# skeskinen/bert.cpp

Hardware: AMD Instinct MI355X
Metric: sentences/sec (seq_len=128) (higher is better)
Workload: dtype f16; 1 GPU; all-MiniLM-L6-v2 f16, batch=256 seq_len=128; per_gpu_batch=256, global_batch=256, seq_len=128, weights=f16, parallelism=dp1 (replicated weights, sharded sentences)

## Files before the change

bert.cpp_amd/csrc/engine.hip:

```cpp
#include "engine.h"

#include <algorithm>
#include <cstdio>
#include <cstdlib>
#include <chrono>
#include <cstring>
#include <system_error>
#include <thread>

namespace bert_hip {

Engine *Engine::create(const ModelFile &mf, int device, std::string &err) {
    int ndev = 0;
    if (hipGetDeviceCount(&ndev) != hipSuccess || ndev <= 0) {
        err = "no HIP device available (this library needs an AMD GPU; there is no CPU fallback)";
        return nullptr;
    }
    if (device < 0 || device >= ndev) { err = "HIP device ordinal " + std::to_string(device) + " out of range"; return nullptr; }
    std::unique_ptr<Engine> e(new Engine);
    e->hp_ = mf.hp;
    e->device_ = device;
    if (hipSetDevice(e->device_) != hipSuccess) { err = "hipSetDevice failed"; return nullptr; }
    hipDeviceProp_t prop;
    if (hipGetDeviceProperties(&prop, e->device_) != hipSuccess) { err = "hipGetDeviceProperties failed"; return nullptr; }
// ... 11 lines not shown
    return e.release();
}

Engine::~Engine() {
    (void)hipSetDevice(device_);
    (void)hipDeviceSynchronize();
    for (auto &sl : slot_) {
        if (sl.h_in) (void)hipHostFree(sl.h_in);
        if (sl.h_out) (void)hipHostFree(sl.h_out);
        if (sl.done) (void)hipEventDestroy(sl.done);
    }
    if (busy_) (void)hipEventDestroy(busy_);
    if (stream_) (void)hipStreamDestroy(stream_);
}

bool Engine::reserve(int n_tokens, int n_sentences, std::string &err) {
    HIP_OK(hipSetDevice(device_), err, false);
    if (n_tokens <= 0 || n_sentences <= 0) return true;
    return ensure_workspace((n_tokens + 255) / 256 * 256, n_sentences, err);
}

int Engine::check(std::string &err) {
    HIP_OK(hipSetDevice(device_), err, -1);
    HIP_OK(hipDeviceSynchronize(), err, -1);
    int st = 0;
    HIP_OK(hipMemcpy(&st, status_.p, sizeof(int), hipMemcpyDeviceToHost), err, -1);
    if (st) HIP_OK(hipMemset(status_.p, 0, sizeof(int)), err, -1);
    return st;
}

void Engine::set_option(const std::string &key, const std::string &value) {
    if (key == "profile_replay") { prof_.set_replay(value); return; }
    (void)hipSetDevice(device_);
    if (!test_poison_option(key, ctx_)) opt_.set(key, value, w_->naive_images(), w_->fold_images);
}

bool Engine::ensure_workspace(int t_pad, int n_sentences, std::string &err) {
    const size_t H = hp_.n_embd, I = hp_.n_intermediate, tp = (size_t)t_pad;
    const size_t es = w_->f32_file ? 4 : 2;
    return x_.ensure(tp * H * es, err) && qkv_.ensure(tp * 3 * H * es, err) && ctx_.ensure(tp * H * es, err) &&
           y_.ensure(tp * H * es, err) && ff_.ensure(tp * I * es, err) && v32_.ensure((size_t)std::max(128, std::min(t_pad, (opt_.latency_tokens + 255) / 256 * 256)) * H * 4, err) &&
           d_out_.ensure((size_t)n_sentences * H * 4, err) &&
           windows_.ensure((size_t)n_sentences * sizeof(int2), err) &&
           (!(H > 384 && H % 256 == 0) || (ln_stats1_.ensure(tp * (2 * H / 256) * 8, err) && ln_stats2_.ensure(tp * (2 * H / 256) * 8, err) &&
                                           ln_rows1_.ensure(tp * 16, err) && ln_rows2_.ensure(tp * 16, err)));
}

void Engine::timed_launch(const char *name, double flops, hipStream_t s, const std::function<void()> &f) { timed(name, flops, s, f); }

std::string Engine::profile_report() {
    (void)hipSetDevice(device_);
    (void)hipDeviceSynchronize();
    return prof_.report();
}

void Engine::build_windows(const int32_t *cu, int B, std::vector<int2> &windows, int slot) {
    windows.clear();
    int first = 0, fill = 0;
    for (int b = 0; b < B; ++b) {
        const int n = cu[b + 1] - cu[b];
        if (b > first && fill + n > 128) {
            windows.push_back(make_int2(first, b - first));
            first = b; fill = 0;
        }
        fill = (fill + n + slot - 1) & ~(slot - 1);
    }
    if (B > first) windows.push_back(make_int2(first, B - first));
// ... 117 lines not shown
    float *v32 = v32_.as<float>();
    for (int il = 0; il < Lz; ++il) {
        const LayerWeights &L = w_->layers[il];
        const LayerWeights *P = il ? &w_->layers[il - 1] : nullptr;
        timed("skinny_qkv", 2.0 * p.T * 3 * H * H, p.s, [&] {
            launch_skinny_gemm(0, L.qkv.w, x, P ? v32 : nullptr, P ? P->ln_out_w.as<float>() : nullptr, P ? P->ln_out_b.as<float>() : nullptr,
                               x, L.qkv_b.as<float>(), nullptr, qkv, nullptr, tb, p.s);
        });
        attention(p);
        timed("skinny_proj", 2.0 * p.T * H * H, p.s, [&] {
            launch_skinny_gemm(1, L.o.w, ctx, nullptr, nullptr, nullptr, nullptr, L.o_b.as<float>(), x, nullptr, v32, tb, p.s);
        });
        timed("skinny_ffn_up", 2.0 * p.T * H * I, p.s, [&] {
            launch_skinny_gemm(2, L.ffi.w, nullptr, v32, L.ln_att_w.as<float>(), L.ln_att_b.as<float>(), y, L.ffi_b.as<float>(), nullptr, ff, nullptr, tb, p.s);
        });
        timed("skinny_ffn_down", 2.0 * p.T * H * I, p.s, [&] {
            launch_skinny_gemm(3, L.ffo.w, ff, nullptr, nullptr, nullptr, nullptr, L.ffo_b.as<float>(), y, nullptr, v32, tb, p.s);
        });
        if (il + 1 == Lz || p.hidden)
            timed("skinny_layernorm", 0.0, p.s, [&] { launch_skinny_layernorm(v32, L.ln_out_w.as<float>(), L.ln_out_b.as<float>(), x, tb, H, p.s); });
        tap(p, il + 1);
    }
}

void Engine::forward_one_launch(const Plan &p) {
    const int H = hp_.n_embd, I = hp_.n_intermediate;
    ModelLayerWeights mw[MODEL_MAX_LAYERS];
    for (int il = 0; il < hp_.n_layer; ++il) {
        const LayerWeights &L = w_->layers[il];
        mw[il] = {&L.qkv.w, &L.o.w, &L.ffi.w, &L.ffo.w, L.qkv_b.as<float>(), L.o_b.as<float>(), L.ln_att_w.as<float>(), L.ln_att_b.as<float>(),
                  L.ffi_b.as<float>(), L.ffo_b.as<float>(), L.ln_out_w.as<float>(), L.ln_out_b.as<float>()};
    }
    timed("model_kernel", hp_.n_layer * (2.0 * p.T * 3 * H * H + 4.0 * p.T * p.max_len * H + 2.0 * p.T * H * H + 4.0 * p.T * H * I), p.s, [&] {
        launch_model_kernel(mw, hp_.n_layer, x_.as<half_t>(), ctx_.as<half_t>(), p.cu, p.B, p.T, p.windows, p.n_windows, p.n_windows_dev, hp_.n_head,
                            p.out, p.max_len, status_.as<int>(), p.pool_mode, p.slots, p.s);
    });
}

bool Engine::forward_folded(const Plan &p, std::string &err) {
    const int H = hp_.n_embd, P = 2 * H / 256;
    const Family G = Family::GEMM256;
    half_t *x = x_.as<half_t>(), *qkv = qkv_.as<half_t>(), *ctx = ctx_.as<half_t>(), *y = y_.as<half_t>(), *ff = ff_.as<half_t>();
    float2 *st1 = ln_stats1_.as<float2>(), *st2 = ln_stats2_.as<float2>();
    float4 *rows1 = ln_rows1_.as<float4>(), *rows2 = ln_rows2_.as<float4>();
    for (int il = 0; il < hp_.n_layer; ++il) {
        const LayerWeights &L = w_->layers[il];
        GemmLnFold ln;
        if (il == 0) {
            if (!gemm(p, "gemm_qkv", G, p.layers[0].planes ? L.qkv_q4 : L.qkv, x, L.qkv_b.as<float>(), nullptr, qkv, EPI_BIAS, err)) return false;
        } else {
            ln.flags = GemmLnFold::IN; ln.rows_in = rows2; ln.waug = L.qkv_waug.as<half_t>();
            if (!gemm(p, "gemm_qkv", G, L.qkv_fold, x, nullptr, nullptr, qkv, EPI_BIAS, err, &ln)) return false;
        }
        attention(p);
        ln = GemmLnFold(); ln.flags = GemmLnFold::STATS | (il ? GemmLnFold::RES : 0); ln.stats = st1; ln.rows_res = rows2; ln.gb = L.o_gb.as<unsigned>();
        if (!gemm(p, "gemm_attn_out", G, L.o, ctx, L.o_b.as<float>(), x, y, EPI_BIAS_RESID, err, &ln)) return false;
        timed("ln_rows_finalize", 0.0, p.s, [&] { launch_ln_rows_finalize(st1, P, p.t_pad, H, rows1, p.s); });
        ln = GemmLnFold(); ln.flags = GemmLnFold::IN; ln.rows_in = rows1; ln.waug = L.ffi_waug.as<half_t>();
        if (!gemm(p, "gemm_ffn_up", G, L.ffi_fold, y, nullptr, nullptr, ff, EPI_BIAS_GELU, err, &ln)) return false;
        ln = GemmLnFold(); ln.flags = GemmLnFold::STATS | GemmLnFold::RES; ln.stats = st2; ln.rows_res = rows1; ln.gb = L.ffo_gb.as<unsigned>();
        if (!gemm(p, "gemm_ffn_down", G, L.ffo, ff, L.ffo_b.as<float>(), y, x, EPI_BIAS_RESID, err, &ln)) return false;
        timed("ln_rows_finalize", 0.0, p.s, [&] { launch_ln_rows_finalize(st2, P, p.t_pad, H, rows2, p.s); });
        if (il + 1 == hp_.n_layer)
            timed("layernorm", 0.0, p.s, [&] { launch_layernorm(x, L.ln_out_w.as<float>(), L.ln_out_b.as<float>(), p.T, H, p.s); });
    }
    return true;
}
// ... 209 lines not shown
```

bert.cpp_amd/csrc/kernels.h:

```cpp
#pragma once
#include <hip/hip_runtime.h>
#include <hip/hip_ext.h>

#include <atomic>
#include <cstdint>
#include <thread>

namespace bert_hip {

typedef _Float16 half_t;

constexpr int GEMM_BM = 128;
constexpr int GEMM_BN = 128;
constexpr int GEMM_BK = 64;

enum Epilogue : int { EPI_BIAS = 0, EPI_BIAS_GELU = 1, EPI_BIAS_RESID = 2 };
enum GemmWType : int { GW_F16 = 0, GW_Q4_0 = 1, GW_Q4_1 = 2 };

struct GemmWeight {
    int N = 0, K = 0, N_pad = 0;
    int type = GW_F16;
    const half_t *w16 = nullptr;
    const uint4 *qs = nullptr;
    const void *sc = nullptr;
    const half_t *naive16 = nullptr;
    const half_t *w16p = nullptr;
    const float *w32 = nullptr;
};

void launch_gemm_mfma(const GemmWeight &W, const half_t *A, const float *bias, const half_t *resid, half_t *C,
                      int M_pad, int epilogue, hipStream_t stream);
bool gemm256_supported(const GemmWeight &W, int M_pad);
struct GemmLnFold {
    enum : int { IN = 1, RES = 2, STATS = 4 };
    int flags = 0;
    const float4 *rows_in = nullptr;
    const half_t *waug = nullptr;
    const float4 *rows_res = nullptr;
    const unsigned *gb = nullptr;
    float2 *stats = nullptr;
};
bool launch_gemm256(const GemmWeight &W, const half_t *A, const float *bias, const half_t *resid, half_t *C, int M_pad,
                    int epilogue, hipStream_t stream, const GemmLnFold *ln = nullptr);
void launch_ln_rows_finalize(const float2 *stats, int P, int T, int H, float4 *rows, hipStream_t stream);
bool layer_tail_supported(const GemmWeight &Wo, const GemmWeight &W1, const GemmWeight &W2);
void launch_layer_tail(const GemmWeight &Wo, const GemmWeight &W1, const GemmWeight &W2, const half_t *ctx, const half_t *x,
                       const float *bo, const float *g1, const float *be1, const float *b1, const float *b2,
                       const float *g2, const float *be2, half_t *out, int M_pad, hipStream_t stream);
constexpr int MODEL_MAX_LAYERS = 12;
struct ModelLayerWeights {
    const GemmWeight *Wqkv, *Wo, *W1, *W2;
    const float *bqkv, *bo, *g1, *be1, *b1, *b2, *g2, *be2;
};
bool model_kernel_supported(const GemmWeight &Wqkv, const GemmWeight &Wo, const GemmWeight &W1, const GemmWeight &W2, int n_layer,
                            int n_head, int d_head, int max_len);
void launch_model_kernel(const ModelLayerWeights *layers, int n_layer, half_t *x, half_t *ctx, const int32_t *cu_seqlens, int n_sentences,
                         int n_tokens, const int2 *groups, int n_groups, const int *n_groups_dev, int n_head, float *pooled, int max_len,
                         int *status, int pool_mode, int slots, hipStream_t stream);
bool skinny_layer_supported(const GemmWeight &Wqkv, const GemmWeight &Wo, const GemmWeight &W1, const GemmWeight &W2);
void launch_skinny_gemm(int mode, const GemmWeight &W, const half_t *A, const float *V, const float *gamma, const float *beta,
                        half_t *ln_out, const float *bias, const half_t *resid, half_t *out16, float *out32, int n_token_blocks,
                        hipStream_t stream);
void launch_skinny_layernorm(const float *v, const float *gamma, const float *beta, half_t *out, int n_token_blocks, int H,
                             hipStream_t stream);
void launch_gemm_naive(const GemmWeight &W, const half_t *A, const float *bias, const half_t *resid, half_t *C,
                       int M, int epilogue, hipStream_t stream);

void launch_embed_ln(const void *word, const void *type, const void *pos, int table_type, const float *gamma,
                     const float *beta, const int32_t *tokens, const int32_t *cu_seqlens, int n_sentences, int T,
                     int H, int n_vocab, int max_len, half_t *out, hipStream_t stream);

void launch_layernorm(half_t *x, const float *gamma, const float *beta, int T, int H, hipStream_t stream);

bool launch_attention_mfma(const half_t *qkv, const int32_t *cu_seqlens, int n_sentences, int n_head, int d_head,
                           int max_len, half_t *out, hipStream_t stream);
void launch_attention_naive(const half_t *qkv, const int32_t *cu_seqlens, int n_sentences, int n_head, int d_head,
                            int max_len, half_t *out, hipStream_t stream);

bool qkv_attention2_supported(const GemmWeight &Wqkv, int n_head, int d_head, int max_len);
int qkv_attention2_sentences_per_window(int max_len, int slots);
void launch_qkv_attention2(const GemmWeight &Wqkv, const half_t *x, const float *bias, const int32_t *cu_seqlens,
                           int n_sentences, const int2 *groups, int n_groups, const int *n_groups_dev, int max_len, int n_head,
                           int slots, half_t *out, hipStream_t stream);
void launch_build_windows(const int32_t *cu_seqlens, int n_sentences, int2 *windows, int *n_windows, int slots, hipStream_t stream);
int qkv_attention2_max_windows(int n_sentences, int n_tokens, int slots);
int window_slots();
void set_window_slots(int slots);

constexpr int POOL_CLS = 1, POOL_RAW = 2;
// ... 51 lines not shown
```

bert.cpp_amd/csrc/layer_tail.hip:

```cpp
#include "device.h"

namespace bert_hip {

namespace {

constexpr int LT_TILE = 16384;
#ifndef LT_ABLATE
#define LT_ABLATE 0
#endif
#ifndef LT_UPRIO
#define LT_UPRIO 1
#endif
#ifndef LT_GELU_BATCH
#define LT_GELU_BATCH 0
#endif
#ifndef LT_DMA_SPLIT
#define LT_DMA_SPLIT 1
#endif
#ifndef LT_DPRIO
#define LT_DPRIO 0
#endif

#ifdef BERT_HIP_TIMELINE
static __device__ unsigned long long g_tl_tail[256 * 512];
// ... 25 lines not shown
    asm volatile("s_waitcnt lgkmcnt(%4)" : "+v"(f[0]), "+v"(f[1]), "+v"(f[2]), "+v"(f[3]) : "n"(N) : "memory");
}
template <int N>
__device__ __forceinline__ void wait_lgkm() {
    asm volatile("s_waitcnt lgkmcnt(%0)" : : "n"(N) : "memory");
}
template <int VM>
__device__ __forceinline__ void close_interval(f16x8 (&f)[4]) {
    asm volatile("s_waitcnt vmcnt(%4) lgkmcnt(0)\n\ts_barrier" : "+v"(f[0]), "+v"(f[1]), "+v"(f[2]), "+v"(f[3]) : "n"(VM) : "memory");
}
template <int OFF>
__device__ __forceinline__ f16x8 frag_read(unsigned addr) {
    if (LT_ABLATE & 4) { f16x8 z = (f16x8)(_Float16)0.f; asm volatile("" : "+v"(z) : "v"(addr)); return z; }
    return lds_read_b128<true, OFF>(addr);
}

__device__ __forceinline__ void dma_m0(unsigned lds) {
    if (LT_ABLATE & 1) return;
    asm volatile("s_mov_b32 m0, %0" : : "s"(lds) : "memory");
}
template <int PIECE>
__device__ __forceinline__ void dma_piece(const char *gbase, unsigned voff) {
    if (LT_ABLATE & 1) return;
    asm volatile("global_load_lds_dwordx4 %0, %1 offset:%2" : : "v"(voff), "s"(gbase - PIECE * 1024), "n"(PIECE * 1024) : "memory");
}

__device__ __forceinline__ f32x16 mfma16(const f16x8 &a, const f16x8 &b, const f32x16 &c) {
    if (LT_ABLATE & 8) { f32x16 r = c; asm volatile("" : "+v"(r[0]) : "v"(a), "v"(b)); return r; }
    return __builtin_amdgcn_mfma_f32_32x32x16_f16(a, b, c, 0, 0, 0);
}

}

template <int NT, int WT, bool RAGGED, bool HANDOVER, bool CTXREGS = false>
__device__ __forceinline__ void layer_tail_body(const TailArgs &a, char *smem, const int tok0, const int rows, const int tid,
                                                [[maybe_unused]] f16x8 (&xnext)[8 * NT], [[maybe_unused]] const f16x8 *cf = nullptr) {
    static_assert(!(HANDOVER && RAGGED), "a ragged window's rows are packed: its lanes are not the window phase's slots");
    static_assert(!(CTXREGS && RAGGED), "a ragged window's rows are packed: its lanes are not the attention waves' queries");
    constexpr bool Q4 = WT != GW_F16;
    constexpr int VMQ = Q4 ? 63 : 0;
    constexpr int H = 128 * NT, NBH = 2 * NT, NB = 4 * NT, NQ = 8 * NT, NYH = 4 * NT;
    constexpr int P = NT * NT;
    constexpr int NG = NT;
    constexpr int LAGT = NT + NG;
    const int I = a.I, NC = I / 64;
    const int lane = tid & 63;
    const int wave = __builtin_amdgcn_readfirstlane(tid >> 6);
    const int t = wave & 3, role = wave >> 2;
    const int l31 = lane & 31, hi = lane >> 5;
    const int tok_w = tok0 + t * 32;
    const int row_l = RAGGED ? tok0 + min(t * 32 + l31, rows - 1) : tok_w + l31;

    char *ringU = smem;
    char *ringD = smem + 3 * LT_TILE;
    char *G = smem + 6 * LT_TILE;
    float *ST = (float *)(G + 32768);
    float *cbo = ST + 8 * 64;
    float *cg1 = cbo + H, *cbe1 = cg1 + H, *cb2 = cbe1 + H, *cg2 = cb2 + H, *cbe2 = cg2 + H, *cb1 = cbe2 + H;

    {
        constexpr int NPB = 4;
        const float *const src[6] = {a.bo, a.g1, a.be1, a.b2, a.g2, a.be2};
        float pv[6];
        f32x4 bq[NPB];
#pragma unroll
        for (int k = 0; k < 6; ++k) pv[k] = tid < H ? src[k][tid] : 0.f;
#pragma unroll
        for (int k = 0; k < NPB; ++k) {
            const int i4 = (k * 512 + tid) * 4;
            bq[k] = i4 < I ? *(const f32x4 *)(a.b1 + i4) : f32x4{0.f, 0.f, 0.f, 0.f};
        }
        if (tid < H) {
#pragma unroll
            for (int k = 0; k < 6; ++k) cbo[k * H + tid] = pv[k];
        }
#pragma unroll
        for (int k = 0; k < NPB; ++k) {
            const int i4 = (k * 512 + tid) * 4;
            if (i4 < I + 128) *(f32x4 *)(cb1 + i4) = bq[k];
        }
    }
    f32x16 accp[NBH];
    f16x4 xv[NBH][4];
    {
        const half_t *xr = a.x + (size_t)row_l * H + role * 64 + 4 * hi;
#pragma unroll
        for (int b = 0; b < NBH; ++b)
#pragma unroll
            for (int gq = 0; gq < 4; ++gq) xv[b][gq] = *(const f16x4 *)(xr + (b >> 1) * 128 + (b & 1) * 32 + 8 * gq);
    }
    f16x8 bf[NQ];
    constexpr bool CTX_LATE = CTXREGS && ctx_edge_offset(NQ) >= 6 * LT_TILE && ctx_edge_offset(NQ) + 16384 <= 6 * LT_TILE + 32768;
    if constexpr (CTXREGS) {
        static_assert(ctx_edge_offset(NQ) >= 5 * LT_TILE && ctx_edge_offset(NQ) + 16384 <= 6 * LT_TILE + 32768,
                      "the edge area: ringD's third slot or G, where the prologue's DMA and parameter writes do not reach");
#pragma unroll
        for (int q = 0; q < NQ - 4; ++q) bf[q] = cf[q];
        const char *const er = smem + ctx_edge_offset(NQ) + t * 4096 + lane * 16;
#pragma unroll
        for (int q = 0; q < (CTX_LATE ? 0 : 4); ++q) bf[NQ - 4 + q] = *(const f16x8 *)(er + q * 1024);
    } else {
        const half_t *cw = a.ctx + (size_t)row_l * H + 8 * hi;
#pragma unroll
        for (int q = 0; q < NQ; ++q) bf[q] = *(const f16x8 *)(cw + 16 * q);
    }

    auto rows_offset = [&](int pitch) __attribute__((always_inline)) {
        int ln = lane;
        asm volatile("" : "+v"(ln));
        const int ch0 = (ln & 7) ^ (ln >> 4), row = t * 32 + (ln >> 3);
        return (unsigned)(row * pitch * 2 + ch0 * 16);
    };
    const half_t *const wo = a.wo, *const w1p = a.w1p, *const w2p = a.w2p;
    auto dma128 = [&](const half_t *base, unsigned oe, int row_bytes, unsigned tile) __attribute__((always_inline)) {
        const char *b = (const char *)base;
        dma_m0(tile + (unsigned)(t * 4096));
        dma_piece<0>(b, oe);
// ... 371 lines not shown
            next_slot();
        };
        using TT = std::true_type; using FF = std::false_type;
        LT_STAMP(tlU, 393);
        __builtin_amdgcn_s_setprio(LT_UPRIO);
        auto u_chunk = [&](auto par_tag, auto first_tag, int c) __attribute__((always_inline)) {
            constexpr bool FIRST = decltype(first_tag)::value;
            static_for<NT>([&](auto j_tag) __attribute__((always_inline)) {
                constexpr int j = decltype(j_tag)::value;
                constexpr bool carry = !(FIRST && j == 0), gelu = !FIRST && j < NG;
                u_interval(par_tag, j_tag, TT{}, std::integral_constant<bool, gelu>{}, std::integral_constant<bool, carry>{}, c);
            });
        };
        u_chunk(std::integral_constant<int, 0>{}, TT{}, 0);
        for (int c = 1; c + 1 < NC; c += 2) {
            u_chunk(std::integral_constant<int, 1>{}, FF{}, c);
            u_chunk(std::integral_constant<int, 0>{}, FF{}, c + 1);
        }
        u_chunk(std::integral_constant<int, 1>{}, FF{}, NC - 1);
        static_for<LAGT>([&](auto k_tag) __attribute__((always_inline)) {
            constexpr int k = decltype(k_tag)::value;
            if constexpr (k < NG)
                u_interval(std::integral_constant<int, 0>{}, std::integral_constant<int, k>{}, FF{}, TT{}, std::integral_constant<bool, k == 0>{}, NC);
            else {
                if constexpr (k == NG) {
                    char *const xu = ringU + t * (NYH * 1024) + lane * 16;
#pragma unroll
                    for (int m = 0; m < NYH; ++m) *(f16x8 *)(xu + m * 1024) = Y[8 * (m >> 2) + (m & 3)];
                }
                pre_close(); dma_barrier<VMQ>(); next_slot();
            }
        });
        static_assert(LAGT > NG, "U needs an idle interval to hand its half of y over");
        asm volatile("s_barrier" ::: "memory");
        asm volatile("s_barrier" ::: "memory");
        store_rows();
        if constexpr (HANDOVER) {
#pragma unroll
            for (int q = 0; q < NQ; ++q) asm volatile("" : "=v"(xnext[q]));
        }
        return;
    } else {
        f16x8 yh[NYH];
        static_for<NBH>([&](auto b_tag) __attribute__((always_inline)) {
            constexpr int b = decltype(b_tag)::value;
            normalise_block(b_tag, yh[2 * b], yh[2 * b + 1]);
            *(f16x8 *)(xch + (2 * b) * 1024) = yh[2 * b];
            *(f16x8 *)(xch + (2 * b + 1) * 1024) = yh[2 * b + 1];
        });
        LT_STAMP(tlD, 400);
        asm volatile("s_waitcnt lgkmcnt(0)\n\ts_barrier" ::: "memory");
        f32x16 acc2[NB];
        static_for<NBH>([&](auto b_tag) __attribute__((always_inline)) {
            constexpr int b = decltype(b_tag)::value, n3 = b >> 1, obp = b & 1;
            f32x4 bu[4], bd[4];
#pragma unroll
            for (int gq = 0; gq < 4; ++gq) {
                bu[gq] = *(const f32x4 *)(cb2 + n3 * 128 + obp * 32 + 8 * gq + 4 * hi);
                bd[gq] = *(const f32x4 *)(cb2 + n3 * 128 + 64 + obp * 32 + 8 * gq + 4 * hi);
            }
#pragma unroll
            for (int gq = 0; gq < 4; ++gq)
#pragma unroll
                for (int e = 0; e < 4; ++e) {
                    acc2[4 * n3 + obp][4 * gq + e] = bu[gq][e];
                    acc2[4 * n3 + 2 + obp][4 * gq + e] = (float)yh[2 * b + (gq >> 1)][4 * (gq & 1) + e] + bd[gq][e];
                }
            asm volatile("" ::: "memory");
        });
// ... 76 lines not shown
                wait_group(N0{}, Fb, gb);
                mm(Fb, gb);
                pre_close();
                dma_barrier<Q4 ? 63 : (up ? 4 : 0) + (dn ? 4 : 0)>();
                next_slot();
            });
        };
        static_assert(LAGT == 2 * NT, "the request schedule below assumes D runs two chunks behind");
        (void)NUP;
        for (int c = 0; c + 3 < NC; ++c) d_chunk(std::integral_constant<int, NT>{}, FF{}, TT{}, c);
        d_chunk(std::integral_constant<int, NT - 2>{}, FF{}, TT{}, NC - 3);
        d_chunk(std::integral_constant<int, 0>{}, FF{}, FF{}, NC - 2);
        d_chunk(std::integral_constant<int, 0>{}, TT{}, FF{}, NC - 1);

        {
            char *S = smem + t * (64 * H);
            int lane = (int)__builtin_amdgcn_mbcnt_hi(~0u, __builtin_amdgcn_mbcnt_lo(~0u, 0u));
            asm volatile("" : "+v"(lane));
            const int hi = lane >> 5;
            {
                const char *const xu = ringU + t * (NYH * 1024) + lane * 16;
#pragma unroll
                for (int n3 = 0; n3 < NT; ++n3) {
                    f16x8 yu[4];
#pragma unroll
                    for (int m = 0; m < 4; ++m) yu[m] = *(const f16x8 *)(xu + (4 * n3 + m) * 1024);
#pragma unroll
                    for (int m = 0; m < 4; ++m)
#pragma unroll
                        for (int e = 0; e < 8; ++e) acc2[4 * n3 + (m >> 1)][8 * (m & 1) + e] += (float)yu[m][e];
                    asm volatile("" ::: "memory");
                }
            }
            asm volatile("s_waitcnt lgkmcnt(0)\n\ts_barrier" ::: "memory");
            float s1 = 0.f, s2 = 0.f;
#pragma unroll
            for (int n = 0; n < NB; ++n)
#pragma unroll
                for (int r = 0; r < 16; ++r) { s1 += acc2[n][r]; s2 = __builtin_fmaf(acc2[n][r], acc2[n][r], s2); }
            s1 += __shfl_xor(s1, 32);
            s2 += __shfl_xor(s2, 32);
            float rstd, nmr;
            layernorm_scale(s1, s2, 1.0f / H, rstd, nmr);
#pragma unroll
            for (int n = 0; n < NB; ++n) {
                f32x4 gv[4], bv[4];
#pragma unroll
                for (int g4 = 0; g4 < 4; ++g4) { gv[g4] = *(const f32x4 *)(cg2 + 32 * n + 8 * g4 + 4 * hi); bv[g4] = *(const f32x4 *)(cbe2 + 32 * n + 8 * g4 + 4 * hi); }
#pragma unroll
                for (int s = 0; s < 2; ++s) {
                    const int q = 2 * n + s;
                    f16x8 o;
#pragma unroll
                    for (int hq = 0; hq < 2; ++hq)
#pragma unroll
                        for (int e = 0; e < 4; ++e)
                            o[4 * hq + e] = (_Float16)rounded_f32(__builtin_fmaf(acc2[n][8 * s + 4 * hq + e], gv[2 * s + hq][e] * rstd, __builtin_fmaf(gv[2 * s + hq][e], nmr, bv[2 * s + hq][e])));
                    *(f16x8 *)(S + q * 1024 + ((lane + 2 * q) & 63) * 16) = o;
                    if constexpr (HANDOVER) xnext[q] = result_to_operand_fragment(o);
                }
                asm volatile("" ::: "memory");
            }
            LT_STAMP(tlD, 401);
            asm volatile("s_waitcnt lgkmcnt(0)\n\ts_barrier" ::: "memory");
        }
        store_rows();
// ... 81 lines not shown
```

bert.cpp_amd/csrc/model_kernel.hip:

```cpp
#define BERT_HIP_PHASES_ONLY
#include "qkv_attention2.hip"
#include "layer_tail.hip"
#undef BERT_HIP_PHASES_ONLY
#include "pool_normalize.h"

#include <cstdlib>

namespace bert_hip {

#ifdef BERT_HIP_MODEL_TIMELINE
static __device__ unsigned long long g_tl_model[1024 * 32];
#define MK_STAMP(i) do { const int mk_i = (i); if (threadIdx.x == 0 && mk_i < 32) g_tl_model[(blockIdx.x & 1023) * 32 + mk_i] = __builtin_amdgcn_s_memrealtime(); } while (0)
#else
#define MK_STAMP(i) do { } while (0)
#endif

namespace {

struct ModelLayerArgs {
    const half_t *wqkv, *wo, *w1p, *w2p;
    const float *bqkv, *bo, *g1, *be1, *b1, *b2, *g2, *be2;
};
struct ModelArgs {
    half_t *x, *ctx;
    const int32_t *cu;
    const int2 *groups;
    const int *n_groups;
    int n_layer, n_head, n_sent, I, slot_mask;
    float *pooled;
    int *status;
    int max_len, pool_mode;
    ModelLayerArgs layer[MODEL_MAX_LAYERS];
};

}

template <int NT, bool RAGGED, bool POOL_MODES>
__global__ __launch_bounds__(512, 2) void model_kernel(ModelArgs m) {
    extern __shared__ __attribute__((aligned(16))) char smem[];
    const int window = (int)blockIdx.x;
    int tok0 = window * 128, rows = 128, first = window, count = 1;
    if constexpr (RAGGED) {
        if (m.groups) {
            if (m.n_groups && window >= *m.n_groups) return;
            const int2 g = m.groups[window];
            first = g.x; count = g.y;
        }
        if (count <= 0 || first >= m.n_sent) return;
        tok0 = m.cu[first];
        rows = min(m.cu[first + count] - tok0, 128);
    }
    const int wave_index = __builtin_amdgcn_readfirstlane((int)threadIdx.x >> 6);
    auto thread_id = [&]() __attribute__((always_inline)) {
        int ln = (int)__builtin_amdgcn_mbcnt_hi(~0u, __builtin_amdgcn_mbcnt_lo(~0u, 0u)), w = wave_index;
        asm volatile("" : "+v"(ln), "+s"(w));
        return w * 64 + ln;
    };
    MK_STAMP(0);
    const int n_layer = rows > 0 ? m.n_layer : 0;
    auto window_phase = [&](const ModelLayerArgs &L, auto xregs_tag, const f16x8 *xf, f16x8 *cf) __attribute__((always_inline)) {
        const int tid = thread_id();
        Qkv2Args q;
        q.x = m.x; q.w = L.wqkv; q.qs = nullptr; q.sc = nullptr; q.bias = L.bqkv; q.cu = m.cu; q.groups = RAGGED ? m.groups : nullptr; q.n_groups = nullptr;
        q.out = m.ctx; q.n_head = m.n_head; q.n_sent = m.n_sent; q.spw = 1; q.slot_mask = m.slot_mask;
        qkv_attention2_body<2 * NT, NT, GW_F16, !RAGGED, decltype(xregs_tag)::value, !RAGGED>(q, smem, window, tid, xf, cf);
    };
    auto tail_phase = [&](const ModelLayerArgs &L, f16x8 (&xf)[8 * NT], const f16x8 *cf) __attribute__((always_inline)) {
        const int tid = thread_id();
        TailArgs t;
        t.ctx = m.ctx; t.x = m.x; t.wo = L.wo; t.w1p = L.w1p; t.w2p = L.w2p;
        t.wo_qs = t.w1_qs = t.w2_qs = nullptr; t.wo_sc = t.w1_sc = t.w2_sc = nullptr;
        t.bo = L.bo; t.g1 = L.g1; t.be1 = L.be1; t.b1 = L.b1; t.b2 = L.b2; t.g2 = L.g2; t.be2 = L.be2; t.out = m.x; t.I = m.I;
        layer_tail_body<NT, GW_F16, RAGGED, !RAGGED, !RAGGED>(t, smem, tok0, rows, tid, xf, cf);
    };
    auto hand_over = [&]() __attribute__((always_inline)) {
        __builtin_amdgcn_fence(__ATOMIC_RELEASE, "workgroup");
        asm volatile("s_waitcnt vmcnt(0) lgkmcnt(0)\n\ts_barrier" ::: "memory");
        __builtin_amdgcn_fence(__ATOMIC_ACQUIRE, "workgroup");
    };
    if constexpr (RAGGED) {
        for (int l = 0; l < n_layer; ++l) {
            f16x8 none[8 * NT];
            window_phase(m.layer[l], std::false_type{}, nullptr, nullptr);
            hand_over();
            MK_STAMP(1 + 2 * l);
            tail_phase(m.layer[l], none, nullptr);
            hand_over();
            MK_STAMP(2 + 2 * l);
        }
    } else {
        f16x8 cf[8 * NT];
        if (n_layer > 0) window_phase(m.layer[0], std::false_type{}, nullptr, cf);
        for (int l = 0; l < n_layer; ++l) {
            hand_over();
            MK_STAMP(1 + 2 * l);
            f16x8 xf[8 * NT];
            tail_phase(m.layer[l], xf, cf);
            hand_over();
            MK_STAMP(2 + 2 * l);
            if (l + 1 < n_layer) window_phase(m.layer[l + 1], std::true_type{}, xf, cf);
            else {
#pragma unroll
                for (int q = 0; q < 8 * NT; ++q) asm volatile("" : "=v"(cf[q]));
            }
        }
    }
    if (m.pooled) {
        const int tid = thread_id();
        for (int j = 0; j < count; ++j) {
            const int b = first + j, t0 = m.cu[b];
            int n = m.cu[b + 1] - t0;
            if (!RAGGED && (t0 != tok0 || n != 128)) n = -1;
            if constexpr (POOL_MODES) pool_normalize_sentence(m.x, t0, n, b, 128 * NT, m.max_len, m.status, m.pooled, (float *)smem, tid, tid < 256, m.pool_mode);
            else pool_normalize_sentence<false, false>(m.x, t0, n, b, 128 * NT, m.max_len, m.status, m.pooled, (float *)smem, tid, tid < 256);
            __syncthreads();
        }
    }
    MK_STAMP(1 + 2 * n_layer);
}

bool model_kernel_supported(const GemmWeight &Wqkv, const GemmWeight &Wo, const GemmWeight &W1, const GemmWeight &W2, int n_layer,
                            int n_head, int d_head, int max_len) {
    const int H = n_head * d_head;
    return n_layer <= MODEL_MAX_LAYERS && (H == 256 || H == 384) && max_len >= 1 && max_len <= 128 &&
           Wqkv.type == GW_F16 && Wo.type == GW_F16 && qkv_attention2_supported(Wqkv, n_head, d_head, max_len) && layer_tail_supported(Wo, W1, W2);
}

void launch_model_kernel(const ModelLayerWeights *layers, int n_layer, half_t *x, half_t *ctx, const int32_t *cu_seqlens, int n_sentences,
                         int n_tokens, const int2 *groups, int n_groups, const int *n_groups_dev, int n_head, float *pooled, int max_len,
                         int *status, int pool_mode, int slots, hipStream_t stream) {
    ModelArgs m;
    m.pooled = pooled; m.status = status; m.max_len = max_len; m.pool_mode = pool_mode;
    m.x = x; m.ctx = ctx; m.cu = cu_seqlens; m.groups = groups; m.n_groups = n_groups_dev;
    m.n_layer = n_layer; m.n_head = n_head; m.n_sent = n_sentences; m.I = layers[0].W1->N; m.slot_mask = slots - 1;
    for (int l = 0; l < n_layer; ++l) {
        const ModelLayerWeights &s = layers[l];
        ModelLayerArgs &d = m.layer[l];
        d.wqkv = s.Wqkv->w16; d.wo = s.Wo->w16; d.w1p = s.W1->w16p; d.w2p = s.W2->w16p;
        d.bqkv = s.bqkv; d.bo = s.bo; d.g1 = s.g1; d.be1 = s.be1; d.b1 = s.b1; d.b2 = s.b2; d.g2 = s.g2; d.be2 = s.be2;
    }
    const int H = layers[0].W1->K, KT = H / 64, GB = KT / 2;
    const size_t lds_q = (size_t)3 * GB * Q2_TILE + 2 * (2 * Q2_WIN * 64 + 32 * Q2_VT_LD * 2) + (size_t)2 * H * sizeof(float);
    const size_t lds = std::max(lds_q, layer_tail_lds(H, m.I));
    const bool full = (long long)n_sentences * 128 == n_tokens;
    if (n_head * 32 != H) { fprintf(stderr, "launch_model_kernel: n_head %d x 32 != H %d\n", n_head, H); abort(); }
    const int grid = full || !groups ? n_sentences : n_groups;
    static DeviceFlags configured[8];
    auto go = [&](auto kernel, int which) {
        configure_once(configured[which], [&] { (void)hipFuncSetAttribute((const void *)kernel, hipFuncAttributeMaxDynamicSharedMemorySize, 160 * 1024); });
        BERT_LAUNCH(kernel, dim3(grid), dim3(512), lds, stream, m);
#ifdef BERT_HIP_MODEL_TIMELINE
        static int shots = 0;
        if (grid >= 256 && shots++ == 30) {
            (void)hipDeviceSynchronize();
            static unsigned long long h[1024 * 32];
            (void)hipMemcpyFromSymbol(h, HIP_SYMBOL(g_tl_model), sizeof(h));
            const int nw = grid < 1024 ? grid : 1024, ns = 2 + 2 * n_layer;
            unsigned long long t0 = ~0ull;
            for (int w = 0; w < nw; ++w) t0 = h[w * 32] < t0 ? h[w * 32] : t0;
            fprintf(stderr, "model_kernel timeline, %d workgroups (us after the first workgroup's start: min mean max):\n", nw);
            for (int i = 0; i < ns; ++i) {
                double lo = 1e30, hi = 0, sum = 0;
                for (int w = 0; w < nw; ++w) { const double v = (double)(h[w * 32 + i] - t0) * 0.01; lo = v < lo ? v : lo; hi = v > hi ? v : hi; sum += v; }
                fprintf(stderr, "  stamp %2d: %8.2f %8.2f %8.2f\n", i, lo, sum / nw, hi);
            }
            fprintf(stderr, "  mean phase durations (window, tail) per layer:");
// ... 34 lines not shown
```

bert.cpp_amd/csrc/options.cpp:

```cpp
#include "options.h"

#include <cstdio>
#include <cstdlib>

#include "weights.h"

namespace bert_hip {

#ifdef BERT_HIP_TEST_ROUTES
static constexpr bool TEST_ROUTES = true;
#else
static constexpr bool TEST_ROUTES = false;
#endif

int EngineOptions::pool_mode() const { return (pool_cls ? POOL_CLS : 0) | (normalize ? 0 : POOL_RAW); }

void EngineOptions::apply(const std::string &key, const std::string &value) {
    const int n = atoi(value.c_str());
    if (key == "pooling" || key == "normalize") {
        const bool pooling = key == "pooling";
        const char *const on = pooling ? "cls" : "1", *const off = pooling ? "mean" : "0";
        if (value == on || value == off) (pooling ? pool_cls : normalize) = value == on;
        else fprintf(stderr, "bert_hip: %s = \"%s\": expected \"%s\" or \"%s\"; ignored\n", key.c_str(), value.c_str(), off, on);
        return;
// ... 13 lines not shown
    else if (key == "chunk_tokens") { if (n > 0) chunk_tokens = n; }
}

EngineOptions EngineOptions::from_env(const HParams &hp) {
    EngineOptions o;
    if (hp.n_embd < 256) o.latency_tokens = 128;
    const std::string kernels = getenv("BERT_HIP_KERNELS") ? getenv("BERT_HIP_KERNELS") : "";
    if (kernels == "naive" && TEST_ROUTES) o.gemm_naive = o.attn_naive = true;
    else if (kernels == "naive") fprintf(stderr, "BERT_HIP_KERNELS=naive: a test cross-check (libbert_test.so), not a route of libbert.so; ignored\n");
    else if (kernels == "tiled") o.qkv2 = o.tail = o.latency = false, o.one_launch = 0;
    if (const char *v = getenv("BERT_HIP_Q4")) o.q4_expand = std::string(v) != "fused";
    static const char *const same_as_key[][2] = {
        {"BERT_HIP_LATENCY", "latency"}, {"BERT_HIP_LATENCY", "latency_tokens"},
        {"BERT_HIP_LN_FOLD", "ln_fold"},
        {"BERT_HIP_CHUNK_TOKENS", "chunk_tokens"}, {"BERT_HIP_WINDOW_SLOTS", "window_slots"},
        {"BERT_HIP_F32", "f32"},
        {"BERT_HIP_POOLING", "pooling"}, {"BERT_HIP_NORMALIZE", "normalize"},
    };
    for (auto &ek : same_as_key)
        if (const char *v = getenv(ek[0])) o.apply(ek[1], v);
    return o;
}

void EngineOptions::set(const std::string &key, const std::string &value, bool naive_images, bool fold_images) {
    if (!TEST_ROUTES && (key == "gemm" || key == "attn") && value == "naive")
        fprintf(stderr, "bert_hip_set_option: %s=naive is a test cross-check (libbert_test.so), not a route of libbert.so; ignored\n", key.c_str());
    else if (key == "gemm" && value == "naive" && !naive_images)
        fprintf(stderr, "bert_hip_set_option: gemm=naive needs BERT_HIP_KERNELS=naive at load time (the f16 row-major images were not built); ignored\n");
    else if (key == "ln_fold" && value != "0" && !fold_images)
        fprintf(stderr, "bert_hip_set_option: ln_fold=1 needs BERT_HIP_LN_FOLD=1 at load time (the folded images were not built); ignored\n");
    else apply(key, value);
}

bool test_poison_option(const std::string &key, const DevBuf &ctx) {
    if (!TEST_ROUTES || key != "test_poison_ctx") return false;
    (void)hipDeviceSynchronize();
    if (ctx.p) (void)hipMemset(ctx.p, 0xFF, ctx.bytes);
    (void)hipDeviceSynchronize();
    return true;
}

}
```

bert.cpp_amd/csrc/options.h:

```cpp
#pragma once
#include <string>

#include "model_file.h"

namespace bert_hip {

struct DevBuf;

struct EngineOptions {
    bool gemm_naive = false, attn_naive = false;
    bool qkv2 = true, gemm256 = true, tail = true;
    bool ln_fold = true;
    bool latency = true;
    bool q4_expand = true;
    bool f32_exact = true;
    int one_launch = 1;
    int chunk_tokens = 262144;
    int latency_tokens = 768;
    bool stage_kernel = true;
    bool pool_cls = false, normalize = true;
    int pool_mode() const;

    static EngineOptions from_env(const HParams &hp);
    void set(const std::string &key, const std::string &value, bool naive_images, bool fold_images);

private:
    void apply(const std::string &key, const std::string &value);
};

bool test_poison_option(const std::string &key, const DevBuf &ctx);

}
```

Baseline: 340,400 sentences/s.

## Keep residual rows in lane-ordered scratch buffer across layers in model kernel

In the one-launch model kernel, the layer tail now writes its LayerNorm output into a per-window scratch buffer (y_) in the lanes' fragment order, and the next layer reads the residual from it directly. This drops the barriers and row-major store_rows pass, and the strided residual gather, on all layers except the first and last. It adds a second residual copy and a poison test hook, and it relies on each full window owning its rows in that lane order.

New measurement: 347,700 sentences/s, median of 6. 1.02x the previous value.

```diff
diff --git a/bert.cpp_amd/csrc/engine.hip b/bert.cpp_amd/csrc/engine.hip
--- a/bert.cpp_amd/csrc/engine.hip
+++ b/bert.cpp_amd/csrc/engine.hip
@@ -67,7 +67,7 @@
 void Engine::set_option(const std::string &key, const std::string &value) {
     if (key == "profile_replay") { prof_.set_replay(value); return; }
     (void)hipSetDevice(device_);
-    if (!test_poison_option(key, ctx_)) opt_.set(key, value, w_->naive_images(), w_->fold_images);
+    if (!test_poison_option(key, ctx_, y_)) opt_.set(key, value, w_->naive_images(), w_->fold_images);
 }
 
 bool Engine::ensure_workspace(int t_pad, int n_sentences, std::string &err) {
@@ -251,7 +251,7 @@
                   L.ffi_b.as<float>(), L.ffo_b.as<float>(), L.ln_out_w.as<float>(), L.ln_out_b.as<float>()};
     }
     timed("model_kernel", hp_.n_layer * (2.0 * p.T * 3 * H * H + 4.0 * p.T * p.max_len * H + 2.0 * p.T * H * H + 4.0 * p.T * H * I), p.s, [&] {
-        launch_model_kernel(mw, hp_.n_layer, x_.as<half_t>(), ctx_.as<half_t>(), p.cu, p.B, p.T, p.windows, p.n_windows, p.n_windows_dev, hp_.n_head,
+        launch_model_kernel(mw, hp_.n_layer, x_.as<half_t>(), ctx_.as<half_t>(), y_.as<half_t>(), p.cu, p.B, p.T, p.windows, p.n_windows, p.n_windows_dev, hp_.n_head,
                             p.out, p.max_len, status_.as<int>(), p.pool_mode, p.slots, p.s);
     });
 }
diff --git a/bert.cpp_amd/csrc/kernels.h b/bert.cpp_amd/csrc/kernels.h
--- a/bert.cpp_amd/csrc/kernels.h
+++ b/bert.cpp_amd/csrc/kernels.h
@@ -54,7 +54,7 @@
 };
 bool model_kernel_supported(const GemmWeight &Wqkv, const GemmWeight &Wo, const GemmWeight &W1, const GemmWeight &W2, int n_layer,
                             int n_head, int d_head, int max_len);
-void launch_model_kernel(const ModelLayerWeights *layers, int n_layer, half_t *x, half_t *ctx, const int32_t *cu_seqlens, int n_sentences,
+void launch_model_kernel(const ModelLayerWeights *layers, int n_layer, half_t *x, half_t *ctx, half_t *xres, const int32_t *cu_seqlens, int n_sentences,
                          int n_tokens, const int2 *groups, int n_groups, const int *n_groups_dev, int n_head, float *pooled, int max_len,
                          int *status, int pool_mode, int slots, hipStream_t stream);
 bool skinny_layer_supported(const GemmWeight &Wqkv, const GemmWeight &Wo, const GemmWeight &W1, const GemmWeight &W2);
diff --git a/bert.cpp_amd/csrc/layer_tail.hip b/bert.cpp_amd/csrc/layer_tail.hip
--- a/bert.cpp_amd/csrc/layer_tail.hip
+++ b/bert.cpp_amd/csrc/layer_tail.hip
@@ -81,11 +81,14 @@
 
 }
 
-template <int NT, int WT, bool RAGGED, bool HANDOVER, bool CTXREGS = false>
+template <int NT, int WT, bool RAGGED, bool HANDOVER, bool CTXREGS = false, bool XRES_IN = false, bool XRES_OUT = false>
 __device__ __forceinline__ void layer_tail_body(const TailArgs &a, char *smem, const int tok0, const int rows, const int tid,
-                                                [[maybe_unused]] f16x8 (&xnext)[8 * NT], [[maybe_unused]] const f16x8 *cf = nullptr) {
+                                                [[maybe_unused]] f16x8 (&xnext)[8 * NT], [[maybe_unused]] const f16x8 *cf = nullptr,
+                                                [[maybe_unused]] half_t *xres = nullptr, const bool lane_in = false, const bool lane_out = false) {
     static_assert(!(HANDOVER && RAGGED), "a ragged window's rows are packed: its lanes are not the window phase's slots");
     static_assert(!(CTXREGS && RAGGED), "a ragged window's rows are packed: its lanes are not the attention waves' queries");
+    static_assert(!((XRES_IN || XRES_OUT) && (RAGGED || WT != GW_F16)), "lane order: full windows (a pair owns its 32 rows), f16 weights");
+    const bool xres_out = XRES_OUT && lane_out;
     constexpr bool Q4 = WT != GW_F16;
     constexpr int VMQ = Q4 ? 63 : 0;
     constexpr int H = 128 * NT, NBH = 2 * NT, NB = 4 * NT, NQ = 8 * NT, NYH = 4 * NT;
@@ -131,7 +134,32 @@
     }
     f32x16 accp[NBH];
     f16x4 xv[NBH][4];
-    {
+    if constexpr (XRES_IN) {
+        char *const xb = (char *)(xres + (size_t)tok_w * H);
+        const unsigned xl = (unsigned)lane * 16u;
+        if (!lane_in) {
+            const half_t *xr = a.x + (size_t)row_l * H + role * 64 + 4 * hi;
+#pragma unroll
+            for (int b = 0; b < NBH; ++b)
+#pragma unroll
+                for (int s = 0; s < 2; ++s) {
+                    const f16x4 lo = *(const f16x4 *)(xr + (b >> 1) * 128 + (b & 1) * 32 + 16 * s), up = *(const f16x4 *)(xr + (b >> 1) * 128 + (b & 1) * 32 + 16 * s + 8);
+                    f16x8 v;
+#pragma unroll
+                    for (int e = 0; e < 4; ++e) { v[e] = lo[e]; v[4 + e] = up[e]; }
+                    *(f16x8 *)(xb + (2 * (4 * (b >> 1) + 2 * role + (b & 1)) + s) * 1024 + xl) = v;
+                }
+            asm volatile("s_waitcnt vmcnt(0)" ::: "memory");
+        }
+#pragma unroll
+        for (int b = 0; b < NBH; ++b)
+#pragma unroll
+            for (int s = 0; s < 2; ++s) {
+                const f16x8 v = *(const f16x8 *)(xb + (2 * (4 * (b >> 1) + 2 * role + (b & 1)) + s) * 1024 + xl);
+#pragma unroll
+                for (int e = 0; e < 4; ++e) { xv[b][2 * s][e] = v[e]; xv[b][2 * s + 1][e] = v[4 + e]; }
+            }
+    } else {
         const half_t *xr = a.x + (size_t)row_l * H + role * 64 + 4 * hi;
 #pragma unroll
         for (int b = 0; b < NBH; ++b)
@@ -569,9 +597,11 @@
             }
         });
         static_assert(LAGT > NG, "U needs an idle interval to hand its half of y over");
-        asm volatile("s_barrier" ::: "memory");
-        asm volatile("s_barrier" ::: "memory");
-        store_rows();
+        if (!xres_out) {
+            asm volatile("s_barrier" ::: "memory");
+            asm volatile("s_barrier" ::: "memory");
+            store_rows();
+        }
         if constexpr (HANDOVER) {
 #pragma unroll
             for (int q = 0; q < NQ; ++q) asm volatile("" : "=v"(xnext[q]));
@@ -714,6 +744,41 @@
                     asm volatile("" ::: "memory");
                 }
             }
+            if constexpr (XRES_OUT) {
+                if (xres_out) {
+                    float s1 = 0.f, s2 = 0.f;
+#pragma unroll
+                    for (int n = 0; n < NB; ++n)
+#pragma unroll
+                        for (int r = 0; r < 16; ++r) { s1 += acc2[n][r]; s2 = __builtin_fmaf(acc2[n][r], acc2[n][r], s2); }
+                    s1 += __shfl_xor(s1, 32);
+                    s2 += __shfl_xor(s2, 32);
+                    float rstd, nmr;
+                    layernorm_scale(s1, s2, 1.0f / H, rstd, nmr);
+                    char *const xb = (char *)(xres + (size_t)tok_w * H);
+                    const unsigned xl = (unsigned)lane * 16u;
+#pragma unroll
+                    for (int n = 0; n < NB; ++n) {
+                        f32x4 gv[4], bv[4];
+#pragma unroll
+                        for (int g4 = 0; g4 < 4; ++g4) { gv[g4] = *(const f32x4 *)(cg2 + 32 * n + 8 * g4 + 4 * hi); bv[g4] = *(const f32x4 *)(cbe2 + 32 * n + 8 * g4 + 4 * hi); }
+#pragma unroll
+                        for (int s = 0; s < 2; ++s) {
+                            const int q = 2 * n + s;
+                            f16x8 o;
+#pragma unroll
+                            for (int hq = 0; hq < 2; ++hq)
+#pragma unroll
+                                for (int e = 0; e < 4; ++e)
+                                    o[4 * hq + e] = (_Float16)rounded_f32(__builtin_fmaf(acc2[n][8 * s + 4 * hq + e], gv[2 * s + hq][e] * rstd, __builtin_fmaf(gv[2 * s + hq][e], nmr, bv[2 * s + hq][e])));
+                            *(f16x8 *)(xb + q * 1024 + xl) = o;
+                            if constexpr (HANDOVER) xnext[q] = result_to_operand_fragment(o);
+                        }
+                        asm volatile("" ::: "memory");
+                    }
+                    return;
+                }
+            }
             asm volatile("s_waitcnt lgkmcnt(0)\n\ts_barrier" ::: "memory");
             float s1 = 0.f, s2 = 0.f;
 #pragma unroll
diff --git a/bert.cpp_amd/csrc/model_kernel.hip b/bert.cpp_amd/csrc/model_kernel.hip
--- a/bert.cpp_amd/csrc/model_kernel.hip
+++ b/bert.cpp_amd/csrc/model_kernel.hip
@@ -31,6 +31,7 @@
     int *status;
     int max_len, pool_mode;
     ModelLayerArgs layer[MODEL_MAX_LAYERS];
+    half_t *xres;
 };
 
 }
@@ -65,13 +66,15 @@
         q.out = m.ctx; q.n_head = m.n_head; q.n_sent = m.n_sent; q.spw = 1; q.slot_mask = m.slot_mask;
         qkv_attention2_body<2 * NT, NT, GW_F16, !RAGGED, decltype(xregs_tag)::value, !RAGGED>(q, smem, window, tid, xf, cf);
     };
-    auto tail_phase = [&](const ModelLayerArgs &L, f16x8 (&xf)[8 * NT], const f16x8 *cf) __attribute__((always_inline)) {
+    auto tail_phase = [&](const ModelLayerArgs &L, f16x8 (&xf)[8 * NT], const f16x8 *cf, [[maybe_unused]] const bool lane_in,
+                          [[maybe_unused]] const bool lane_out) __attribute__((always_inline)) {
         const int tid = thread_id();
         TailArgs t;
         t.ctx = m.ctx; t.x = m.x; t.wo = L.wo; t.w1p = L.w1p; t.w2p = L.w2p;
         t.wo_qs = t.w1_qs = t.w2_qs = nullptr; t.wo_sc = t.w1_sc = t.w2_sc = nullptr;
         t.bo = L.bo; t.g1 = L.g1; t.be1 = L.be1; t.b1 = L.b1; t.b2 = L.b2; t.g2 = L.g2; t.be2 = L.be2; t.out = m.x; t.I = m.I;
-        layer_tail_body<NT, GW_F16, RAGGED, !RAGGED, !RAGGED>(t, smem, tok0, rows, tid, xf, cf);
+        if constexpr (RAGGED) layer_tail_body<NT, GW_F16, true, false, false>(t, smem, tok0, rows, tid, xf, cf);
+        else layer_tail_body<NT, GW_F16, false, true, true, true, true>(t, smem, tok0, rows, tid, xf, cf, m.xres, lane_in, lane_out);
     };
     auto hand_over = [&]() __attribute__((always_inline)) {
         __builtin_amdgcn_fence(__ATOMIC_RELEASE, "workgroup");
@@ -84,7 +87,7 @@
             window_phase(m.layer[l], std::false_type{}, nullptr, nullptr);
             hand_over();
             MK_STAMP(1 + 2 * l);
-            tail_phase(m.layer[l], none, nullptr);
+            tail_phase(m.layer[l], none, nullptr, false, false);
             hand_over();
             MK_STAMP(2 + 2 * l);
         }
@@ -95,7 +98,7 @@
             hand_over();
             MK_STAMP(1 + 2 * l);
             f16x8 xf[8 * NT];
-            tail_phase(m.layer[l], xf, cf);
+            tail_phase(m.layer[l], xf, cf, l > 0, l + 1 < n_layer);
             hand_over();
             MK_STAMP(2 + 2 * l);
             if (l + 1 < n_layer) window_phase(m.layer[l + 1], std::true_type{}, xf, cf);
@@ -126,12 +129,12 @@
            Wqkv.type == GW_F16 && Wo.type == GW_F16 && qkv_attention2_supported(Wqkv, n_head, d_head, max_len) && layer_tail_supported(Wo, W1, W2);
 }
 
-void launch_model_kernel(const ModelLayerWeights *layers, int n_layer, half_t *x, half_t *ctx, const int32_t *cu_seqlens, int n_sentences,
+void launch_model_kernel(const ModelLayerWeights *layers, int n_layer, half_t *x, half_t *ctx, half_t *xres, const int32_t *cu_seqlens, int n_sentences,
                          int n_tokens, const int2 *groups, int n_groups, const int *n_groups_dev, int n_head, float *pooled, int max_len,
                          int *status, int pool_mode, int slots, hipStream_t stream) {
     ModelArgs m;
     m.pooled = pooled; m.status = status; m.max_len = max_len; m.pool_mode = pool_mode;
-    m.x = x; m.ctx = ctx; m.cu = cu_seqlens; m.groups = groups; m.n_groups = n_groups_dev;
+    m.x = x; m.ctx = ctx; m.xres = xres; m.cu = cu_seqlens; m.groups = groups; m.n_groups = n_groups_dev;
     m.n_layer = n_layer; m.n_head = n_head; m.n_sent = n_sentences; m.I = layers[0].W1->N; m.slot_mask = slots - 1;
     for (int l = 0; l < n_layer; ++l) {
         const ModelLayerWeights &s = layers[l];
diff --git a/bert.cpp_amd/csrc/options.cpp b/bert.cpp_amd/csrc/options.cpp
--- a/bert.cpp_amd/csrc/options.cpp
+++ b/bert.cpp_amd/csrc/options.cpp
@@ -69,10 +69,11 @@
     else apply(key, value);
 }
 
-bool test_poison_option(const std::string &key, const DevBuf &ctx) {
-    if (!TEST_ROUTES || key != "test_poison_ctx") return false;
+bool test_poison_option(const std::string &key, const DevBuf &ctx, const DevBuf &xres) {
+    if (!TEST_ROUTES || (key != "test_poison_ctx" && key != "test_poison_xres")) return false;
+    const DevBuf &buf = key == "test_poison_ctx" ? ctx : xres;
     (void)hipDeviceSynchronize();
-    if (ctx.p) (void)hipMemset(ctx.p, 0xFF, ctx.bytes);
+    if (buf.p) (void)hipMemset(buf.p, 0xFF, buf.bytes);
     (void)hipDeviceSynchronize();
     return true;
 }
diff --git a/bert.cpp_amd/csrc/options.h b/bert.cpp_amd/csrc/options.h
--- a/bert.cpp_amd/csrc/options.h
+++ b/bert.cpp_amd/csrc/options.h
@@ -28,6 +28,6 @@
     void apply(const std::string &key, const std::string &value);
 };
 
-bool test_poison_option(const std::string &key, const DevBuf &ctx);
+bool test_poison_option(const std::string &key, const DevBuf &ctx, const DevBuf &xres);
 
 }
```
